# powdr-labs/powdr

Measured on AMD Instinct MI355X. Metric: STARK cells/sec (trace rows x cols) proving guest-keccak [bus interactions (LogUp) inside the proof], higher is better.
Workload: dtype u32 (BabyBear, Montgomery)

## Files before the change

powdr_amd/csrc/babybear.hpp:

```cpp
#pragma once
#if defined(__HIPCC_RTC__)
using __hip_internal::int32_t;
using __hip_internal::int64_t;
using __hip_internal::uint8_t;
using __hip_internal::uint32_t;
using __hip_internal::uint64_t;
#else
#include <stdint.h>
#endif

#if defined(__HIPCC__)
#if !defined(__HIPCC_RTC__)
#include <hip/hip_runtime.h>
#endif
#define PW_HD __host__ __device__ __forceinline__
#else
#define PW_HD inline
#endif

namespace bb {

constexpr uint32_t P = 0x78000001u;
constexpr uint32_t NEG_PINV = 0x77ffffffu;
constexpr uint32_t R_MOD_P = 0x0ffffffeu;
// ... 19 lines not shown
    uint32_t m = (uint32_t)t * NEG_PINV;
    uint64_t u = t + (uint64_t)m * P;
    return (uint32_t)(u >> 32);
}
PW_HD uint32_t add_loose(uint32_t a, uint32_t b) { return reduce_2p(a + b); }
PW_HD uint32_t mul(uint32_t a, uint32_t b) { return monty_reduce((uint64_t)a * b); }
PW_HD uint32_t mul2(uint32_t a, uint32_t b, uint32_t c, uint32_t d) { return monty_reduce((uint64_t)a * b + (uint64_t)c * d); }
PW_HD uint32_t sqr(uint32_t a) { return mul(a, a); }

PW_HD uint32_t to_monty(uint32_t canonical) { return mul(canonical, R2_MOD_P); }
PW_HD uint32_t from_monty(uint32_t x) { return monty_reduce((uint64_t)x); }

PW_HD uint32_t mul_lazy(uint32_t a, uint32_t b) {
    uint64_t t = (uint64_t)a * b;
    uint32_t m = (uint32_t)t * NEG_PINV;
    uint64_t u = t + (uint64_t)m * P;
    return (uint32_t)(u >> 32);
}

PW_HD uint64_t wide_add(uint64_t acc, uint32_t x) {
#if defined(__HIP_DEVICE_COMPILE__)
    uint64_t out;
    asm("v_mad_u64_u32 %0, vcc, %1, 1, %2" : "=v"(out) : "v"(x), "v"(acc) : "vcc");
    return out;
#else
    return acc + x;
#endif
}
PW_HD uint64_t wide_fma(uint64_t acc, uint32_t x, uint32_t k) {
#if defined(__HIP_DEVICE_COMPILE__)
    uint64_t out;
    asm("v_mad_u64_u32 %0, vcc, %1, %2, %3" : "=v"(out) : "v"(x), "n"(k), "v"(acc) : "vcc");
    return out;
#else
    return acc + (uint64_t)x * k;
#endif
}
PW_HD uint64_t wide_fma_uniform(uint64_t c, uint32_t x, uint32_t k) {
#if defined(__HIP_DEVICE_COMPILE__)
    uint64_t out;
    asm("v_mad_u64_u32 %0, vcc, %1, %2, %3" : "=v"(out) : "v"(x), "n"(k), "s"(c) : "vcc");
    return out;
#else
    return c + (uint64_t)x * k;
#endif
}
PW_HD uint64_t wide_mad_uniform(uint64_t acc, uint32_t x, uint32_t u) {
#if defined(__HIP_DEVICE_COMPILE__)
    uint64_t out;
    asm("v_mad_u64_u32 %0, vcc, %1, %2, %3" : "=v"(out) : "v"(x), "s"(u), "v"(acc) : "vcc");
    return out;
#else
    return acc + (uint64_t)x * u;
#endif
}
PW_HD uint64_t wide_mul(uint32_t x, uint32_t k) {
#if defined(__HIP_DEVICE_COMPILE__)
    uint64_t out;
    asm("v_mad_u64_u32 %0, vcc, %1, %2, 0" : "=v"(out) : "v"(x), "n"(k) : "vcc");
    return out;
#else
    return (uint64_t)x * k;
#endif
}
PW_HD uint32_t reduce_wide_loose(uint64_t x) {
    const uint32_t q = (uint32_t)(((x >> 7) & 0xffffffffull) * 273u >> 32);
#if defined(__HIP_DEVICE_COMPILE__) && !defined(PW_NO_REDUCE_MAD)
    uint64_t out;
    asm("v_mad_u64_u32 %0, vcc, %1, %2, %3" : "=v"(out) : "v"(q), "s"(0u - P), "v"(x) : "vcc");
    return (uint32_t)out;
#else
    return (uint32_t)x - q * P;
#endif
}
PW_HD uint32_t reduce_wide(uint64_t x) { return reduce_2p(reduce_wide_loose(x)); }
PW_HD uint32_t reduce_sum(uint64_t x) {
    const uint32_t q = (uint32_t)(x >> 31);
    return reduce_2p((uint32_t)x - q * P);
}

PW_HD int64_t smul(int32_t a, int32_t b) {
#if defined(__HIP_DEVICE_COMPILE__)
    int64_t out;
    asm("v_mad_i64_i32 %0, vcc, %1, %2, 0" : "=v"(out) : "v"(a), "v"(b) : "vcc");
    return out;
#else
    return (int64_t)a * b;
#endif
}
PW_HD int64_t smul_uniform(int32_t a, int32_t u) {
#if defined(__HIP_DEVICE_COMPILE__)
    int64_t out;
    asm("v_mad_i64_i32 %0, vcc, %1, %2, 0" : "=v"(out) : "v"(a), "s"(u) : "vcc");
    return out;
#else
    return (int64_t)a * u;
#endif
}
PW_HD int32_t smont(int64_t t) {
    const int32_t m = (int32_t)((uint32_t)t * NEG_PINV);
#if defined(__HIP_DEVICE_COMPILE__)
    int64_t u;
    asm("v_mad_i64_i32 %0, vcc, %1, %2, %3" : "=v"(u) : "v"(m), "s"((int32_t)P), "v"(t) : "vcc");
    return (int32_t)(u >> 32);
#else
    return (int32_t)((t + (int64_t)m * (int64_t)P) >> 32);
#endif
}
PW_HD int64_t swide_add(int64_t acc, int32_t x) {
#if defined(__HIP_DEVICE_COMPILE__)
    int64_t out;
    asm("v_mad_i64_i32 %0, vcc, %1, 1, %2" : "=v"(out) : "v"(x), "v"(acc) : "vcc");
    return out;
#else
    return acc + x;
#endif
}
PW_HD int64_t swide_fma(int64_t acc, int32_t x, int32_t k) {
#if defined(__HIP_DEVICE_COMPILE__)
    int64_t out;
    asm("v_mad_i64_i32 %0, vcc, %1, %2, %3" : "=v"(out) : "v"(x), "n"(k), "v"(acc) : "vcc");
    return out;
#else
    return acc + (int64_t)x * k;
#endif
}
PW_HD int64_t swide_fma_uniform(int64_t c, int32_t x, int32_t k) {
#if defined(__HIP_DEVICE_COMPILE__)
    int64_t out;
    asm("v_mad_i64_i32 %0, vcc, %1, %2, %3" : "=v"(out) : "v"(x), "n"(k), "s"(c) : "vcc");
    return out;
#else
    return c + (int64_t)x * k;
#endif
}
PW_HD int64_t swide_mad_uniform(int64_t acc, int32_t x, int32_t u) {
#if defined(__HIP_DEVICE_COMPILE__)
    int64_t out;
    asm("v_mad_i64_i32 %0, vcc, %1, %2, %3" : "=v"(out) : "v"(x), "s"(u), "v"(acc) : "vcc");
    return out;
#else
    return acc + (int64_t)x * u;
#endif
}
PW_HD int64_t swide_mul(int32_t x, int32_t k) {
#if defined(__HIP_DEVICE_COMPILE__)
    int64_t out;
    asm("v_mad_i64_i32 %0, vcc, %1, %2, 0" : "=v"(out) : "v"(x), "n"(k) : "vcc");
    return out;
#else
    return (int64_t)x * k;
#endif
}
PW_HD int32_t sreduce_wide_loose(int64_t y) {
    const int32_t a = (int32_t)(y >> 7);
    const int32_t q = (int32_t)(((int64_t)a * 273) >> 32);
#if defined(__HIP_DEVICE_COMPILE__)
    int64_t out;
    asm("v_mad_i64_i32 %0, vcc, %1, %2, %3" : "=v"(out) : "v"(q), "s"(-(int32_t)P), "v"(y) : "vcc");
    return (int32_t)out;
#else
    return (int32_t)((uint32_t)y - (uint32_t)q * P);
#endif
}
PW_HD int32_t centred(uint32_t canonical) { return canonical > P / 2 ? (int32_t)(canonical - P) : (int32_t)canonical; }
PW_HD uint32_t canonical_of(int32_t x) {
    uint32_t u = (uint32_t)x;
    u = umin(u, u + P);
    return umin(u, u - P);
}

constexpr uint32_t TWO_P = 2u * P;
PW_HD uint32_t add_2p(uint32_t a, uint32_t b) {
    const uint32_t s = a + b;
    const uint32_t t = s - TWO_P;
    return s < a ? t : umin(s, t);
}
PW_HD uint32_t sub_2p(uint32_t a, uint32_t b) {
    const uint32_t d = a - b;
    return a < b ? d + TWO_P : d;
}

PW_HD uint32_t double_(uint32_t a) { return add(a, a); }
PW_HD uint32_t halve(uint32_t a) {
    uint32_t t = (a & 1u) ? a + P : a;
    return t >> 1;
}

PW_HD uint32_t pow_u32(uint32_t a, uint32_t e) {
    uint32_t r = R_MOD_P;
    while (e) {
        if (e & 1u) r = mul(r, a);
        a = sqr(a);
        e >>= 1;
    }
    return r;
}

PW_HD uint32_t inv(uint32_t a) {
    uint32_t x2 = sqr(a);
    uint32_t x3 = mul(x2, a);
    uint32_t x6 = sqr(x3);
    uint32_t x7 = mul(x6, a);
    uint32_t o3 = x7;
    uint32_t o6 = o3;
    for (int i = 0; i < 3; ++i) o6 = sqr(o6);
    o6 = mul(o6, o3);
    uint32_t o12 = o6;
    for (int i = 0; i < 6; ++i) o12 = sqr(o12);
    o12 = mul(o12, o6);
    uint32_t o24 = o12;
    for (int i = 0; i < 12; ++i) o24 = sqr(o24);
    o24 = mul(o24, o12);
    uint32_t o27 = o24;
    for (int i = 0; i < 3; ++i) o27 = sqr(o27);
    o27 = mul(o27, o3);
    uint32_t hi = x7;
    for (int i = 0; i < 28; ++i) hi = sqr(hi);
    return mul(hi, o27);
}
PW_HD uint32_t inv_or_zero(uint32_t a) { return a == 0 ? 0u : inv(a); }

}
```

powdr_amd/csrc/ntt.hip:

```cpp
#include "babybear.hpp"
#include "common.hpp"
#include "prover_internal.hpp"

#include <cstdlib>
#include <map>
#include <mutex>
#include <tuple>
#include <type_traits>
#include <vector>

namespace pw {

namespace {

constexpr int kBlock = 256;
__constant__ uint32_t c_roots16[2][8];

__global__ void fill_powers_kernel(uint32_t* out, uint32_t base, uint32_t scale, size_t n) {
    size_t i = (size_t)blockIdx.x * blockDim.x + threadIdx.x;
    if (i < n) out[i] = bb::mul(bb::pow_u32(base, (uint32_t)i), scale);
}
__global__ void bitrev_copy_kernel(const uint32_t* in, uint32_t* out, int n) {
    size_t i = (size_t)blockIdx.x * blockDim.x + threadIdx.x;
    if (i >= ((size_t)1 << n)) return;
// ... 232 lines not shown
                }
            }
        } else {
#pragma unroll
            for (int rho = 0; rho < R; ++rho) tile[p0 + lds_off(rho)] = x[rho];
        }
    }
}

template <bool DIF, int LOGT, int MODE, bool TWT = false>
__global__ __launch_bounds__(kBlock) void ntt_group_kernel(const uint32_t* __restrict__ in, uint32_t* __restrict__ out,
                                                           size_t in_stride, size_t out_stride, GroupParams gp,
                                                           const uint32_t* __restrict__ tw,
                                                           const uint32_t* __restrict__ scale_br) {
    constexpr int EPT = (1 << LOGT) / kBlock;
    __shared__ uint32_t tile[(1 << LOGT) + ((1 << LOGT) >> 5)];
    const int tid = threadIdx.x;
    IndexMap im;
    im.B = gp.B; im.c = gp.c; im.lowbits = gp.lowbits; im.k = gp.k;
    im.cmask = (1u << gp.c) - 1u;
    im.tile0 = (size_t)blockIdx.x << (LOGT - gp.B);
    im.n_tiles = (size_t)gp.n_tiles;
    const uint32_t* src = in + (size_t)blockIdx.y * in_stride;
    uint32_t* dst = out + (size_t)blockIdx.y * out_stride;
    uint32_t tw_base = TWT ? 0u : load_twiddle_base<DIF>(im, gp, 0, 0, tid, tw);
    constexpr bool kStageFold = MODE == 2;
    const bool select = MODE == 2 && gp.n_sel > 0;
    if (kStageFold) {
        if (gp.B == LOGT && gp.c == 0 && gp.lowbits == 0 && gp.fold <= 1) {
            const size_t g0 = (size_t)blockIdx.x << LOGT;
            constexpr int kVec = (1 << LOGT) / (4 * kBlock);
            if (gp.fold == 0) {
                const uint4* pv = reinterpret_cast<const uint4*>(src + g0);
                uint4 d[kVec];
#pragma unroll
                for (int m = 0; m < kVec; ++m) d[m] = pv[(uint32_t)tid + kBlock * m];
                const uint32_t k0 = gp.foldk[0];
#pragma unroll
                for (int m = 0; m < kVec; ++m) {
                    const uint32_t l = 4u * ((uint32_t)tid + kBlock * m);
                    tile[lds_phys(l)] = bb::mul(d[m].x, k0); tile[lds_phys(l + 1)] = bb::mul(d[m].y, k0);
                    tile[lds_phys(l + 2)] = bb::mul(d[m].z, k0); tile[lds_phys(l + 3)] = bb::mul(d[m].w, k0);
                }
            } else {
                const uint4* pv = reinterpret_cast<const uint4*>(src + 2 * g0);
                uint4 d[2 * kVec];
#pragma unroll
                for (int m = 0; m < 2 * kVec; ++m) d[m] = pv[(uint32_t)tid + kBlock * m];
                const uint32_t k0 = gp.foldk[0], k1 = gp.foldk[1];
#pragma unroll
                for (int m = 0; m < 2 * kVec; ++m) {
                    const uint32_t l = 2u * ((uint32_t)tid + kBlock * m);
                    tile[lds_phys(l)] = bb::mul2(d[m].x, k0, d[m].y, k1);
                    tile[lds_phys(l + 1)] = bb::mul2(d[m].z, k0, d[m].w, k1);
                }
            }
        } else {
#pragma unroll 4
            for (uint32_t l = (uint32_t)tid; l < (1u << LOGT); l += kBlock) {
                bool valid;
                const size_t g = im.global(l, valid);
                tile[lds_phys(l)] = valid ? fold_load(src, gp.foldk, g, gp.fold) : 0u;
            }
        }
        __syncthreads();
    }
    for (int r = 0; r < gp.n_rounds; ++r) {
        switch (gp.logr[r]) {
            case 1: run_round<DIF, 1, EPT, MODE, TWT>(tile, im, gp, r, src, dst, tw, scale_br, tid, tw_base, !kStageFold, !select); break;
            case 2: run_round<DIF, 2, EPT, MODE, TWT>(tile, im, gp, r, src, dst, tw, scale_br, tid, tw_base, !kStageFold, !select); break;
            case 3: run_round<DIF, 3, EPT, MODE, TWT>(tile, im, gp, r, src, dst, tw, scale_br, tid, tw_base, !kStageFold, !select); break;
            default: run_round<DIF, 4, EPT, MODE, TWT>(tile, im, gp, r, src, dst, tw, scale_br, tid, tw_base, !kStageFold, !select); break;
        }
        if (r + 1 < gp.n_rounds) __syncthreads();
    }
    if (select) {
        __syncthreads();
        const size_t t = blockIdx.x;
        uint32_t* part = gp.sel_part ? gp.sel_part + ((size_t)blockIdx.y * gp.n_tiles + t) * (size_t)gp.n_sel : nullptr;
        for (int q = tid; q < gp.n_sel; q += kBlock) {
            const uint32_t v = bb::reduce_2p(tile[lds_phys(gp.sel_pos[q])]);
            const uint32_t term = bb::mul(v, gp.sel_xpow[(size_t)q * gp.n_tiles + t]);
            if (part) part[q] = term;
            else atomicAdd(gp.sel_acc + (size_t)blockIdx.y * gp.n_sel + q, (unsigned long long)term);
        }
    }
}

template <bool DIF, int EPT, bool TWT = false>
__device__ __forceinline__ void run_group(uint32_t* tile, const IndexMap& im, const GroupParams& gp, const uint32_t* __restrict__ src,
                                          uint32_t* __restrict__ dst, const uint32_t* __restrict__ tw, int tid, bool io_first, bool io_last) {
    uint32_t tw_base = TWT ? 0u : load_twiddle_base<DIF>(im, gp, 0, 0, tid, tw);
    for (int r = 0; r < gp.n_rounds; ++r) {
        switch (gp.logr[r]) {
            case 1: run_round<DIF, 1, EPT, 0, TWT>(tile, im, gp, r, src, dst, tw, nullptr, tid, tw_base, io_first, io_last); break;
            case 2: run_round<DIF, 2, EPT, 0, TWT>(tile, im, gp, r, src, dst, tw, nullptr, tid, tw_base, io_first, io_last); break;
            case 3: run_round<DIF, 3, EPT, 0, TWT>(tile, im, gp, r, src, dst, tw, nullptr, tid, tw_base, io_first, io_last); break;
            default: run_round<DIF, 4, EPT, 0, TWT>(tile, im, gp, r, src, dst, tw, nullptr, tid, tw_base, io_first, io_last); break;
        }
        if (r + 1 < gp.n_rounds) __syncthreads();
    }
}

__global__ __launch_bounds__(kBlock) void lde_fused_kernel(const uint32_t* __restrict__ in, uint32_t* __restrict__ out, size_t in_stride,
                                                           size_t out_stride, GroupParams ga, GroupParams gd,
                                                           const uint32_t* __restrict__ tw_inv, const uint32_t* __restrict__ tw_fwd,
                                                           const uint32_t* __restrict__ scale_br) {
    constexpr int LOGA = 12, LOGD = 13;
    __shared__ uint32_t tile[(1 << LOGD) + ((1 << LOGD) >> 5)];
    const int tid = threadIdx.x;
    const uint32_t* src = in + (size_t)blockIdx.y * in_stride;
    uint32_t* dst = out + (size_t)blockIdx.y * out_stride;
    IndexMap ia;
    ia.B = ga.B; ia.c = ga.c; ia.lowbits = ga.lowbits; ia.k = ga.k;
    ia.cmask = (1u << ga.c) - 1u;
    ia.tile0 = (size_t)blockIdx.x << (LOGA - ga.B);
    ia.n_tiles = (size_t)ga.n_tiles;
    run_group<true, (1 << LOGA) / kBlock, true>(tile, ia, ga, src, nullptr, tw_inv, tid, true, false);
    __syncthreads();
    uint32_t v[(1 << LOGA) / kBlock];
#pragma unroll
    for (int m = 0; m < (1 << LOGA) / kBlock; ++m) {
        const uint32_t l = (uint32_t)tid + 256u * m;
        bool valid;
        const size_t q = ia.global(l, valid);
        const uint32_t sc = valid ? scale_br[q] : 0u;
        v[m] = bb::mul(tile[lds_phys(l)], sc);
    }
    __syncthreads();
#pragma unroll
    for (int m = 0; m < (1 << LOGA) / kBlock; ++m) {
        const uint32_t l = (uint32_t)tid + 256u * m;
        tile[lds_phys(2 * l)] = v[m];
        tile[lds_phys(2 * l + 1)] = v[m];
    }
    __syncthreads();
    IndexMap id;
    id.B = gd.B; id.c = gd.c; id.lowbits = gd.lowbits; id.k = gd.k;
    id.cmask = (1u << gd.c) - 1u;
    id.tile0 = (size_t)blockIdx.x << (LOGD - gd.B);
    id.n_tiles = (size_t)gd.n_tiles;
    run_group<false, (1 << LOGD) / kBlock, true>(tile, id, gd, nullptr, dst, tw_fwd, tid, false, true);
}

constexpr uint32_t kF12A0 = 0, kF12A1 = 15u * 256u, kF12A2 = kF12A1 + 15u * 16u;
constexpr uint32_t kF12D0 = 4096, kF12D1 = kF12D0 + 15u * 2u, kF12D2 = kF12D1 + 15u * 32u;
constexpr uint32_t kF12Words = kF12D2 + 15u * 512u;

template <int RB>
__device__ constexpr uint32_t f12_off(int rho) {
    return ((uint32_t)rho << RB) + (RB >= 5 ? ((uint32_t)rho << (RB >= 5 ? RB - 5 : 0)) : ((uint32_t)rho >> (RB >= 5 ? 0 : 5 - RB)));
}

template <bool CANON>
__global__ __launch_bounds__(kBlock) void lde_fused12_kernel(const uint32_t* __restrict__ in, uint32_t* __restrict__ out, size_t in_stride,
                                                             size_t out_stride, const uint32_t* __restrict__ tw, uint32_t hinv) {
    __shared__ uint32_t tile[(1 << 13) + ((1 << 13) >> 5)];
    const uint32_t tid = threadIdx.x;
    const uint32_t* src = in + (size_t)blockIdx.y * in_stride + ((size_t)blockIdx.x << 12);
    uint32_t* dst = out + (size_t)blockIdx.y * out_stride + ((size_t)blockIdx.x << 13);
    uint32_t x[16], tt[16], tn[16];
#pragma unroll
    for (int rho = 0; rho < 16; ++rho) x[rho] = src[tid + 256u * rho];
#pragma unroll
    for (int j = 0; j < 15; ++j) tt[j] = tw[kF12A0 + 256u * j + tid];
#pragma unroll
    for (int j = 0; j < 15; ++j) tn[j] = tw[kF12A1 + 16u * j + (tid & 15u)];
    slot_butterflies<true, 4, true>(x, 0u, tt);
    {
        const uint32_t p0 = lds_phys(tid);
#pragma unroll
        for (int rho = 0; rho < 16; ++rho) tile[p0 + f12_off<8>(rho)] = x[rho];
    }
    __syncthreads();
    {
        const uint32_t k = ((tid >> 5) & 1u) | (((tid >> 4) & 1u) << 1) | ((tid >> 6) << 2);
        const uint32_t p0 = lds_phys((k << 8) | (tid & 15u));
#pragma unroll
        for (int rho = 0; rho < 16; ++rho) x[rho] = tile[p0 + f12_off<4>(rho)];
        slot_butterflies<true, 4, true>(x, 0u, tn);
#pragma unroll
        for (int rho = 0; rho < 16; ++rho) tile[p0 + f12_off<4>(rho)] = x[rho];
    }
    __syncthreads();
    {
        const uint32_t p0 = lds_phys(tid << 4);
#pragma unroll
        for (int rho = 0; rho < 16; ++rho) x[rho] = tile[p0 + (uint32_t)rho];
#pragma unroll
        for (int j = 0; j < 15; ++j) tn[j] = tw[kF12D1 + 32u * j + (tid & 31u)];
#pragma unroll
        for (int j = 0; j < 15; ++j) tt[j] = tw[kF12A2 + j];
        slot_butterflies<true, 4, true>(x, 0u, tt);
#pragma unroll
        for (int rho = 0; rho < 16; ++rho) x[rho] = bb::mul(x[rho], hinv);
    }
    __syncthreads();
    {
        const uint32_t p0 = lds_phys(tid << 5);
#pragma unroll
        for (int b = 0; b < 2; ++b) {
            uint32_t y[16];
#pragma unroll
            for (int rho = 0; rho < 16; ++rho) y[rho] = x[rho];
#pragma unroll
            for (int j = 0; j < 15; ++j) tt[j] = tw[kF12D0 + 2u * j + b];
            slot_butterflies<false, 4, true>(y, 0u, tt);
#pragma unroll
            for (int rho = 0; rho < 16; ++rho) tile[p0 + 2u * rho + b] = y[rho];
        }
    }
    __syncthreads();
    uint32_t tf[2][16];
#pragma unroll
    for (int m = 0; m < 2; ++m) {
#pragma unroll
        for (int j = 0; j < 15; ++j) tf[m][j] = tw[kF12D2 + 512u * j + tid + 256u * m];
    }
#pragma unroll
    for (int m = 0; m < 2; ++m) {
        const uint32_t sigma = tid + 256u * m;
        const uint32_t p0 = lds_phys(((sigma >> 5) << 9) | (sigma & 31u));
#pragma unroll
        for (int rho = 0; rho < 16; ++rho) x[rho] = tile[p0 + f12_off<5>(rho)];
        slot_butterflies<false, 4, true>(x, 0u, tn);
#pragma unroll
        for (int rho = 0; rho < 16; ++rho) tile[p0 + f12_off<5>(rho)] = x[rho];
    }
    __syncthreads();
#pragma unroll
    for (int m = 0; m < 2; ++m) {
        const uint32_t sigma = tid + 256u * m;
        const uint32_t p0 = lds_phys(sigma);
#pragma unroll
        for (int rho = 0; rho < 16; ++rho) x[rho] = tile[p0 + f12_off<9>(rho)];
        slot_butterflies<false, 4, true>(x, 0u, tf[m]);
#pragma unroll
        for (int rho = 0; rho < 16; ++rho) dst[sigma + 512u * rho] = CANON ? bb::reduce_2p(x[rho]) : x[rho];
    }
}

template <int RB>
__device__ __forceinline__ constexpr uint32_t strided8_words(int lb, int m, int rho) {
    return RB == 9 ? (((uint32_t)(8 * m) << lb) + ((uint32_t)rho << (lb + 4))) : (((uint32_t)m << (lb + 7)) + ((uint32_t)rho << lb));
}
typedef __attribute__((address_space(1))) const char* GlobalBytesIn;
typedef __attribute__((address_space(1))) char* GlobalBytesOut;
__device__ __forceinline__ uint32_t ld_off4(const uint32_t* base, uint32_t off4) {
    GlobalBytesIn b = (GlobalBytesIn)base;
    asm("" : "+s"(b));
    return *(__attribute__((address_space(1))) const uint32_t*)(b + off4);
}
__device__ __forceinline__ void st_off4(uint32_t* base, uint32_t off4, uint32_t v) {
    GlobalBytesOut b = (GlobalBytesOut)base;
    asm("" : "+s"(b));
    *(__attribute__((address_space(1))) uint32_t*)(b + off4) = v;
}

template <bool DIF, int K>
__global__ __launch_bounds__(kBlock) void ntt_strided_kernel(const uint32_t* in, uint32_t* out, size_t in_stride, size_t out_stride,
                                                             const uint32_t* __restrict__ tw, uint32_t cst_lo, uint32_t cst_hi) {
    static_assert(K == 8, "the 2^20-row geometry; other heights take ntt_group_kernel");
    constexpr int LB = DIF ? 12 : 13;
    constexpr int RB0 = DIF ? 9 : 5, RB1 = DIF ? 5 : 9;
    __shared__ uint32_t tile[(1 << 13) + ((1 << 13) >> 5)];
    const uint32_t tid = threadIdx.x, row = tid >> 5, col = tid & 31u;
    const size_t t0 = (size_t)blockIdx.x << 5;
    const uint32_t* src = in + (size_t)blockIdx.y * in_stride + t0;
    uint32_t* dst = out + (size_t)blockIdx.y * out_stride + t0;
    const uint32_t off_hi = 4u * ((row << LB) | col), off_lo = 4u * ((row << (LB + 4)) | col);
    const uint32_t off0 = RB0 == 9 ? off_hi : off_lo, off1 = RB1 == 9 ? off_hi : off_lo;
    uint32_t x[2][16];
#pragma unroll
    for (int m = 0; m < 2; ++m) {
#pragma unroll
        for (int rho = 0; rho < 16; ++rho) x[m][rho] = ld_off4(src + strided8_words<RB0>(LB, m, rho), off0);
    }
    uint32_t b_hi[2], b_lo;
#pragma unroll
    for (int m = 0; m < 2; ++m) b_hi[m] = ld_off4(tw + t0 + ((uint32_t)(8 * m) << LB), off_hi);
    b_lo = ld_off4(tw + (t0 << 4), col << 6);
    if (!DIF) {
        b_lo = bb::mul(b_lo, cst_lo);
#pragma unroll
        for (int m = 0; m < 2; ++m) b_hi[m] = bb::mul(b_hi[m], cst_hi);
    }
    const uint32_t p_hi = lds_phys(tid), p_lo = (row << 9) + (row << 4) + col;
    const uint32_t p0 = RB0 == 9 ? p_hi : p_lo, p1 = RB1 == 9 ? p_hi : p_lo;
    constexpr uint32_t kSlot0 = RB0 == 9 ? 264u : 4224u, kSlot1 = RB1 == 9 ? 264u : 4224u;
#pragma unroll
    for (int m = 0; m < 2; ++m) {
        slot_butterflies<DIF, 4>(x[m], RB0 == 9 ? b_hi[m] : b_lo);
#pragma unroll
        for (int rho = 0; rho < 16; ++rho) tile[p0 + kSlot0 * m + f12_off<RB0>(rho)] = x[m][rho];
    }
    __syncthreads();
#pragma unroll
    for (int m = 0; m < 2; ++m) {
        uint32_t y[16];
#pragma unroll
        for (int rho = 0; rho < 16; ++rho) y[rho] = tile[p1 + kSlot1 * m + f12_off<RB1>(rho)];
        slot_butterflies<DIF, 4>(y, RB1 == 9 ? b_hi[m] : b_lo);
#pragma unroll
        for (int rho = 0; rho < 16; ++rho) st_off4(dst + strided8_words<RB1>(LB, m, rho), off1, DIF ? y[rho] : bb::reduce_2p(y[rho]));
    }
}

struct Tables {
    uint32_t* tw_fwd = nullptr;
    uint32_t* tw_inv = nullptr;
    uint32_t* shift = nullptr;
    uint32_t* shift_br = nullptr;
};
std::mutex g_mu;
std::map<std::pair<int, int>, Tables> g_tables;
uint64_t g_roots_uploaded = 0;

int upload_roots() {
    int device = 0;
    PW_HIP_TRY(hipGetDevice(&device));
    if (device < 64 && (g_roots_uploaded >> device) & 1) return 0;
    uint32_t h[2][8];
    const uint32_t w16 = field::root_of_unity(4), w16i = bb::inv(w16);
    uint32_t a = bb::R_MOD_P, b = bb::R_MOD_P;
    for (int r = 0; r < 8; ++r) { h[0][r] = a; h[1][r] = b; a = bb::mul(a, w16); b = bb::mul(b, w16i); }
    PW_HIP_TRY(hipMemcpyToSymbol(HIP_SYMBOL(c_roots16), h, sizeof h));
    if (device < 64) g_roots_uploaded |= 1ull << device;
    return 0;
}

const Tables* tables(int n) {
    std::lock_guard<std::mutex> lk(g_mu);
    if (upload_roots()) return nullptr;
    int device = 0;
    if (hipGetDevice(&device) != hipSuccess) return nullptr;
    const std::pair<int, int> key{device, n};
    auto it = g_tables.find(key);
    if (it != g_tables.end()) return &it->second;
    Tables t;
    size_t half = n ? (size_t)1 << (n - 1) : 1, full = (size_t)1 << n;
    if (hipMalloc(&t.tw_fwd, half * 4) != hipSuccess) return nullptr;
    if (hipMalloc(&t.tw_inv, half * 4) != hipSuccess) return nullptr;
    if (hipMalloc(&t.shift, full * 4) != hipSuccess) return nullptr;
    if (hipMalloc(&t.shift_br, full * 4) != hipSuccess) return nullptr;
    uint32_t w = field::root_of_unity(n);
    uint32_t one = bb::R_MOD_P;
    hipLaunchKernelGGL(fill_powers_kernel, dim3(div_up(half, 256)), dim3(256), 0, stream(), t.tw_fwd, w, one, half);
    hipLaunchKernelGGL(fill_powers_kernel, dim3(div_up(half, 256)), dim3(256), 0, stream(), t.tw_inv, bb::inv(w), one, half);
    uint32_t ninv = bb::inv(bb::to_monty((uint32_t)(((uint64_t)1 << n) % bb::P)));
    hipLaunchKernelGGL(fill_powers_kernel, dim3(div_up(full, 256)), dim3(256), 0, stream(), t.shift,
                       bb::to_monty(field::kCosetShift), ninv, full);
    hipLaunchKernelGGL(bitrev_copy_kernel, dim3(div_up(full, 256)), dim3(256), 0, stream(), t.shift, t.shift_br, n);
    if (hipStreamSynchronize(stream()) != hipSuccess) return nullptr;
    return &g_tables.emplace(key, t).first->second;
}

GroupParams make_group(bool dif, int n, int s, int k, int c) {
    GroupParams g{};
    g.n = n; g.s0 = s; g.k = k; g.c = c; g.lowbits = dif ? n - s - k : s; g.B = k + c;
    g.n_tiles = 1ull << (n - g.B);
    int nr = (k + 3) / 4;
    g.n_rounds = nr;
    int widths[4];
    for (int r = 0; r < nr; ++r) widths[r] = k / nr + (r < k % nr ? 1 : 0);
    if (dif) {
        int top = c + k;
        for (int r = 0; r < nr; ++r) { top -= widths[r]; g.rb[r] = top; g.logr[r] = widths[r]; }
    } else {
        int bot = c;
        for (int r = 0; r < nr; ++r) { g.rb[r] = bot; g.logr[r] = widths[r]; bot += widths[r]; }
    }
    return g;
}

std::vector<GroupParams> plan_groups(bool dif, int n, int first, int& logt_out, int end = -1, bool balance = false) {
    std::vector<GroupParams> out;
    int kStridedC = (n - (dif ? 0 : 1)) >= 18 ? 5 : 4;
    if (const char* e = getenv("POWDR_NTT_C")) { int v = atoi(e); if (v >= 0 && v <= 6) kStridedC = v; }
    if (end < 0) end = n;
    const int total = end - first;
    int logt = 12;
    int n_groups = 0;
    {
        auto passes = [&](int lt) {
            int s = first, p = 0;
            while (s < end) {
                int rem = end - s, k = rem < lt ? rem : lt;
                for (; k >= 1; --k) { int lb = dif ? n - s - k : s; int c = lb < kStridedC ? lb : kStridedC; if (k + c <= lt) break; }
                s += k; ++p;
            }
            return p;
// ... 76 lines not shown
    const unsigned j = (i - a.off[r]) >> a.rb[r];
    const int q = 31 - __clz((int)(j + 1));
    out[i] = bb::mul(tab[i], a.cq[r][q]);
}

struct CosetSpec {
    int fold_log;
    uint32_t foldk[16];
    uint32_t C[32];
    uint32_t* d_scratch;
    int n_sel = 0;
    const uint32_t* sel_pos = nullptr;
    const uint32_t* sel_xpow = nullptr;
    unsigned long long* sel_acc = nullptr;
    uint32_t* sel_part = nullptr;
};

template <class Launch>
void for_column_chunks(uint32_t cols, Launch&& launch) {
    for (uint32_t c0 = 0; c0 < cols; c0 += 65535u) launch(c0, cols - c0 < 65535u ? cols - c0 : 65535u);
}

template <bool DIF>
void launch_group_kernel(int logt, int mode, dim3 grid, const uint32_t* src, uint32_t* dst, size_t src_stride, size_t dst_stride,
                         const GroupParams& g, const uint32_t* table, const uint32_t* tw, const uint32_t* scale_br) {
    auto launch = [&](auto lt, auto md) {
        constexpr int LT = decltype(lt)::value, MD = decltype(md)::value;
        if (table) hipLaunchKernelGGL((ntt_group_kernel<DIF, LT, MD, true>), grid, dim3(kBlock), 0, stream(), src, dst, src_stride, dst_stride, g, table, scale_br);
        else hipLaunchKernelGGL((ntt_group_kernel<DIF, LT, MD, false>), grid, dim3(kBlock), 0, stream(), src, dst, src_stride, dst_stride, g, tw, scale_br);
    };
    auto with_mode = [&](auto lt) {
        if constexpr (!DIF) {
            if (mode == 2) return launch(lt, std::integral_constant<int, 2>{});
            if (mode == 1) return launch(lt, std::integral_constant<int, 1>{});
        }
        launch(lt, std::integral_constant<int, 0>{});
    };
    if (logt == 13) with_mode(std::integral_constant<int, 13>{});
    else with_mode(std::integral_constant<int, 12>{});
}

template <bool DIF>
bool strided8_geometry(const GroupParams& g, int logt) {
    return logt == 13 && g.n == (DIF ? 20 : 21) && g.s0 == (DIF ? 0 : 13) && g.k == 8 && g.c == 5 && g.lowbits == (DIF ? 12 : 13) && g.B == 13 &&
           g.n_tiles == (DIF ? 128ull : 256ull) && g.n_rounds == 2 && g.logr[0] == 4 && g.logr[1] == 4 && g.rb[0] == (DIF ? 9 : 5) &&
           g.rb[1] == (DIF ? 5 : 9) && (DIF || g.canonical_out) && !g.fold && !g.n_sel;
}

template <bool DIF>
void launch_groups(std::vector<GroupParams>& groups, int logt, int mode, const uint32_t* in, uint32_t* out, size_t in_stride, size_t out_stride,
                   uint32_t cols, const uint32_t* tw, const uint32_t* expand_scale_br, const char* name, const CosetSpec* cs = nullptr,
                   const uint32_t* coset_pw = nullptr, bool fused_schedule = false) {
    const uint32_t* src = in;
    size_t src_stride = in_stride;
    for (auto& g : groups) {
        const unsigned wgs = (unsigned)div_up((size_t)g.n_tiles, (size_t)1 << (logt - g.B));
        const GroupTwiddles* gt = group_twiddles(g, DIF);
        if (gt) for (int r = 0; r < 4; ++r) g.twt_off[r] = gt->off[r];
        const uint32_t* table = gt ? gt->d : nullptr;
        if (coset_pw) {
            g.coset = 1;
            for (int r = 0; r < g.n_rounds; ++r) g.cst[r] = coset_pw[g.n - 1 - (g.s0 + g.rb[r] + g.logr[r] - 1 - g.c)];
        }
        if (cs) {
            g.coset = 1;
            g.fold = mode == 2 ? cs->fold_log : 0;
            for (int k = 0; k < 16; ++k) g.foldk[k] = cs->foldk[k];
            if (mode == 2 && cs->n_sel > 0) { g.n_sel = cs->n_sel; g.sel_pos = cs->sel_pos; g.sel_xpow = cs->sel_xpow; g.sel_acc = cs->sel_acc; g.sel_part = cs->sel_part; }
            for (int r = 0; r < g.n_rounds; ++r) g.cst[r] = cs->C[g.s0 + g.rb[r] + g.logr[r] - 1 - g.c];
            if (gt) {
                CosetTableArgs a{};
                a.n_rounds = g.n_rounds;
                for (int r = 0; r < g.n_rounds; ++r) {
                    a.off[r] = gt->off[r]; a.rb[r] = g.rb[r]; a.logr[r] = g.logr[r];
                    for (int q = 0; q < g.logr[r]; ++q) a.cq[r][q] = cs->C[g.s0 + g.rb[r] - g.c + q];
                }
                const int lr = g.n_rounds - 1;
                a.total = gt->off[lr] + (((1u << g.logr[lr]) - 1u) << g.rb[lr]);
                hipLaunchKernelGGL(coset_table_kernel, dim3(div_up(a.total, 256)), dim3(256), 0, stream(), gt->d, cs->d_scratch, a);
                table = cs->d_scratch;
            }
        }
        if (fused_schedule && mode == 0 && !table && !cs && strided8_geometry<DIF>(g, logt)) {
            const uint32_t one = bb::R_MOD_P;
            const uint32_t cst_lo = g.coset ? g.cst[DIF ? 1 : 0] : one, cst_hi = g.coset ? g.cst[DIF ? 0 : 1] : one;
            for_column_chunks(cols, [&](uint32_t c0, uint32_t cc) {
                ScopedKernelTimer t(name);
                call_stats()[kStatNttStridedFixedLaunches] += 1;
                hipLaunchKernelGGL((ntt_strided_kernel<DIF, 8>), dim3((unsigned)g.n_tiles, cc), dim3(kBlock), 0, stream(), src + (size_t)c0 * src_stride,
                                   out + (size_t)c0 * out_stride, src_stride, out_stride, tw, cst_lo, cst_hi);
            });
            src = out;
            src_stride = out_stride;
            continue;
        }
        for_column_chunks(cols, [&](uint32_t c0, uint32_t cc) {
            ScopedKernelTimer t(mode == 2 ? "ntt_subcoset_first_group_kernel" : name);
            launch_group_kernel<DIF>(logt, mode, dim3(wgs, cc), src + (size_t)c0 * src_stride, out + (size_t)c0 * out_stride, src_stride, out_stride,
                                     g, table, tw, expand_scale_br);
        });
        src = out;
        src_stride = out_stride;
        mode = 0;
        expand_scale_br = nullptr;
    }
}

template <bool DIF>
void run_groups(const uint32_t* in, uint32_t* out, size_t in_stride, size_t out_stride, uint32_t cols, int n,
                int first_stage, const uint32_t* tw, const uint32_t* expand_scale_br, const char* name, const CosetSpec* cs = nullptr,
                int max_groups = -1, int* stages_done = nullptr) {
    int logt = 12;
    auto groups = plan_groups(DIF, n, first_stage, logt);
    if (max_groups >= 0 && (size_t)max_groups < groups.size()) groups.resize((size_t)max_groups);
    if (stages_done) { *stages_done = first_stage; for (auto& g : groups) *stages_done += g.k; }
    const bool complete = !stages_done || *stages_done == n;
    if (!groups.empty() && complete) groups.back().canonical_out = 1;
    launch_groups<DIF>(groups, logt, cs ? 2 : expand_scale_br != nullptr ? 1 : 0, in, out, in_stride, out_stride, cols, tw, expand_scale_br, name, cs);
    if (groups.empty() && in != out) {
        for (uint32_t c = 0; c < cols; ++c)
            (void)hipMemcpyAsync(out + (size_t)c * out_stride, in + (size_t)c * in_stride, (size_t)4 << n,
                                 hipMemcpyDeviceToDevice, stream());
    }
}

__global__ void expand_small_kernel(const uint32_t* in, uint32_t* out, size_t in_stride, size_t out_stride, size_t h,
                                    const uint32_t* scale_br) {
    size_t q = (size_t)blockIdx.x * blockDim.x + threadIdx.x;
    if (q >= h) return;
    uint32_t v = bb::mul(in[(size_t)blockIdx.y * in_stride + q], scale_br[q]);
    out[(size_t)blockIdx.y * out_stride + 2 * q] = v;
    out[(size_t)blockIdx.y * out_stride + 2 * q + 1] = v;
}

struct FusedTwiddles {
    uint32_t* d = nullptr;
    unsigned dif_off[4] = {0, 0, 0, 0}, dit_off[4] = {0, 0, 0, 0};
    size_t dit_base = 0;
};
std::map<std::pair<int, int>, FusedTwiddles> g_fused_tw;

const FusedTwiddles* fused_twiddles(int ka, const GroupParams& ga, const GroupParams& gd) {
    return cached_table(g_fused_tw, ka, [&](std::vector<uint32_t>& h, FusedTwiddles& ft) {
        append_group_table(h, ga, true, ft.dif_off, 0);
        ft.dit_base = h.size();
        append_group_table(h, gd, false, ft.dit_off, ft.dit_base);
        return true;
    });
}

struct Fused12Twiddles { uint32_t* d = nullptr; };
std::map<std::pair<int, int>, Fused12Twiddles> g_fused12_tw;

const uint32_t* fused12_twiddles(int n, const GroupParams& ga, const GroupParams& gd, const uint32_t* pw) {
    const Fused12Twiddles* ft = cached_table(g_fused12_tw, n, [&](std::vector<uint32_t>& h, Fused12Twiddles&) {
        unsigned dif_off[4] = {0, 0, 0, 0}, dit_off[4] = {0, 0, 0, 0};
        append_group_table(h, ga, true, dif_off, 0);
        if (h.size() > kF12D0) return false;
        h.resize(kF12D0, 0u);
        append_group_table(h, gd, false, dit_off, kF12D0);
        if (dif_off[0] != kF12A0 || dif_off[1] != kF12A1 || dif_off[2] != kF12A2 || dit_off[0] != 0 || kF12D0 + dit_off[1] != kF12D1 ||
            kF12D0 + dit_off[2] != kF12D2 || h.size() != kF12Words)
            return false;
        for (int r = 0; r < gd.n_rounds; ++r) {
            const size_t G = (size_t)1 << gd.rb[r];
            uint32_t* tab = h.data() + kF12D0 + dit_off[r];
            for (int q = 0; q < gd.logr[r]; ++q) {
                const uint32_t cq = pw[n - (gd.s0 + gd.rb[r] - gd.c + q)];
                for (size_t i = (((size_t)1 << q) - 1) * G; i < (((size_t)2 << q) - 1) * G; ++i) tab[i] = bb::mul(tab[i], cq);
            }
        }
        return true;
    });
    return ft ? ft->d : nullptr;
}

}

int lde_fused(const uint32_t* in, uint32_t* tmp, uint32_t* out, size_t in_stride, size_t tmp_stride, size_t out_stride, uint32_t cols, int n) {
    if (n == 0) {
        int rc = intt_dif(in, tmp, in_stride, tmp_stride, cols, n);
        return rc ? rc : coset_lde_from_coeffs(tmp, out, tmp_stride, out_stride, cols, n);
    }
    const Tables* tn = tables(n);
    const Tables* t1 = tables(n + 1);
    if (!tn || !t1) return (int)hipErrorOutOfMemory;
    const int ka = n < 12 ? n : 12;
    const char* force_generic = getenv("POWDR_LDE_FUSED_GENERIC");
    const bool spec12 = ka == 12 && !(force_generic && atoi(force_generic) != 0);
    const char* strided_generic = getenv("POWDR_NTT_STRIDED_GENERIC");
    const bool strided_fixed = !(strided_generic && atoi(strided_generic) != 0);
    const uint32_t hinv = bb::inv(bb::to_monty((uint32_t)(((uint64_t)1 << n) % bb::P)));
    const uint32_t* src = in;
    size_t src_stride = in_stride;
    if (n > ka) {
        int logt = 12;
        auto groups = plan_groups(true, n, 0, logt, n - ka, true);
        launch_groups<true>(groups, logt, 0, in, tmp, in_stride, tmp_stride, cols, tn->tw_inv, nullptr, "ntt_group_kernel<dif>", nullptr, nullptr,
                            strided_fixed);
        src = tmp;
        src_stride = tmp_stride;
    }
    GroupParams ga = make_group(true, n, n - ka, ka, 0);
    GroupParams gd = make_group(false, n + 1, 1, ka, 1);
    gd.canonical_out = ka == n ? 1 : 0;
    uint32_t coset_pw[33];
    if (spec12) {
        coset_pw[0] = bb::to_monty(field::kCosetShift);
        for (int e = 1; e <= n; ++e) coset_pw[e] = bb::sqr(coset_pw[e - 1]);
        const uint32_t* tw12 = fused12_twiddles(n, ga, gd, coset_pw);
        if (!tw12) return (int)hipErrorOutOfMemory;
        const unsigned wgs = 1u << (n - 12);
        for_column_chunks(cols, [&](uint32_t c0, uint32_t cc) {
            ScopedKernelTimer t("lde_fused_kernel");
            const uint32_t* s_ = src + (size_t)c0 * src_stride;
            uint32_t* d_ = out + (size_t)c0 * out_stride;
            if (n == 12) hipLaunchKernelGGL(lde_fused12_kernel<true>, dim3(wgs, cc), dim3(kBlock), 0, stream(), s_, d_, src_stride, out_stride, tw12, hinv);
            else hipLaunchKernelGGL(lde_fused12_kernel<false>, dim3(wgs, cc), dim3(kBlock), 0, stream(), s_, d_, src_stride, out_stride, tw12, hinv);
        });
    } else {
        const FusedTwiddles* ft = fused_twiddles(ka, ga, gd);
        if (!ft) return (int)hipErrorOutOfMemory;
        for (int r = 0; r < 4; ++r) { ga.twt_off[r] = ft->dif_off[r]; gd.twt_off[r] = ft->dit_off[r]; }
        const unsigned wgs = (unsigned)div_up((size_t)ga.n_tiles, (size_t)1 << (12 - ka));
        for_column_chunks(cols, [&](uint32_t c0, uint32_t cc) {
            ScopedKernelTimer t("lde_fused_kernel");
            hipLaunchKernelGGL(lde_fused_kernel, dim3(wgs, cc), dim3(kBlock), 0, stream(), src + (size_t)c0 * src_stride,
                               out + (size_t)c0 * out_stride, src_stride, out_stride, ga, gd, ft->d, ft->d + ft->dit_base, tn->shift_br);
        });
    }
    if (n > ka) {
        int logt = 12;
        auto groups = plan_groups(false, n + 1, ka + 1, logt, n + 1, true);
        if (!groups.empty()) groups.back().canonical_out = 1;
        launch_groups<false>(groups, logt, 0, out, out, out_stride, out_stride, cols, t1->tw_fwd, nullptr, "ntt_group_kernel<dit>", nullptr,
                             spec12 ? coset_pw : nullptr, strided_fixed);
    }
    return (int)hipGetLastError();
}

int intt_dif(const uint32_t* in, uint32_t* out, size_t in_stride, size_t out_stride, uint32_t cols, int n) {
    const Tables* t = tables(n);
    if (!t) return (int)hipErrorOutOfMemory;
    run_groups<true>(in, out, in_stride, out_stride, cols, n, 0, t->tw_inv, nullptr, "ntt_group_kernel<dif>");
    return (int)hipGetLastError();
}

int coset_lde_from_coeffs(const uint32_t* coeffs, uint32_t* out, size_t in_stride, size_t out_stride, uint32_t cols, int n) {
    const Tables* tn = tables(n);
    const Tables* t1 = tables(n + 1);
    if (!tn || !t1) return (int)hipErrorOutOfMemory;
    if (n == 0) {
        ScopedKernelTimer t("expand_small_kernel");
        hipLaunchKernelGGL(expand_small_kernel, dim3(1, cols), dim3(64), 0, stream(), coeffs, out, in_stride, out_stride,
                           (size_t)1, tn->shift_br);
        return (int)hipGetLastError();
    }
    run_groups<false>(coeffs, out, in_stride, out_stride, cols, n + 1, 1, t1->tw_fwd, tn->shift_br, "ntt_group_kernel<dit>");
    return (int)hipGetLastError();
}

namespace {
bool subcoset_spec(int n, int b, uint32_t r, uint32_t* d_scratch, CosetSpec& cs) {
    const int nm = n + 1 - b;
    if (b < 1 || b > 5 || nm < 1 || (r >> b)) return false;
    cs = CosetSpec{};
    cs.fold_log = b - 1;
    cs.d_scratch = d_scratch;
    uint32_t pw[32];
    pw[0] = bb::mul(bb::to_monty(field::kCosetShift), bb::pow_u32(field::root_of_unity(n + 1), r));
    for (int e = 1; e <= nm; ++e) pw[e] = bb::sqr(pw[e - 1]);
    for (int s = 0; s < nm; ++s) cs.C[s] = pw[nm - 1 - s];
    const uint32_t hinv = bb::inv(bb::to_monty((uint32_t)(((uint64_t)1 << n) % bb::P)));
    const int f = b - 1;
    for (uint32_t tp = 0; tp < (1u << f); ++tp) {
        const uint32_t t = f ? (__builtin_bitreverse32(tp) >> (32 - f)) : 0u;
        cs.foldk[tp] = bb::mul(bb::pow_u32(pw[nm], t), hinv);
    }
    return true;
}

__global__ __launch_bounds__(256) void subcoset_rows_kernel(const uint32_t* __restrict__ part, size_t stride, uint32_t cols, int k1, int k2, uint32_t c0,
                                                            uint32_t wm, const uint32_t* __restrict__ idx, const uint32_t* __restrict__ slot,
                                                            uint32_t* __restrict__ out) {
    const uint32_t c = blockIdx.x * 256u + threadIdx.x;
    if (c >= cols) return;
    const uint32_t i = idx[blockIdx.y];
    const uint32_t x = bb::mul(c0, bb::pow_u32(wm, i));
    const uint32_t* col = part + (size_t)c * stride + (i & ((1u << k1) - 1u));
    uint32_t acc = 0u, xp = bb::R_MOD_P;
    for (uint32_t u = 0; u < (1u << k2); ++u) {
        const uint32_t t = k2 ? (__brev(u) >> (32 - k2)) : 0u;
        acc = bb::add(acc, bb::mul(bb::reduce_2p(col[(size_t)t << k1]), xp));
        xp = bb::mul(xp, x);
    }
    out[(size_t)(slot ? slot[blockIdx.y] : blockIdx.y) * cols + c] = acc;
}
__global__ __launch_bounds__(256) void select_xpow_kernel(const uint32_t* __restrict__ idx, uint32_t n_idx, int k2, uint32_t c0, uint32_t wm,
                                                         uint32_t* __restrict__ xpow, uint32_t* __restrict__ pos, uint32_t pos_mask) {
    const size_t gid = (size_t)blockIdx.x * 256 + threadIdx.x;
    const size_t n_tiles = (size_t)1 << k2;
    if (gid >= (size_t)n_idx * n_tiles) return;
    const uint32_t q = (uint32_t)(gid >> k2), t = (uint32_t)(gid & (n_tiles - 1));
    const uint32_t i = idx[q];
    const uint32_t x = bb::mul(c0, bb::pow_u32(wm, i));
    const uint32_t u = k2 ? (__brev(t) >> (32 - k2)) : 0u;
    xpow[gid] = bb::pow_u32(x, u);
    if (t == 0) pos[q] = i & pos_mask;
}

__global__ __launch_bounds__(256) void select_finish_kernel(const unsigned long long* __restrict__ acc, uint32_t n, uint32_t cols,
                                                           const uint32_t* __restrict__ slot, uint32_t* __restrict__ out) {
    const uint32_t c = blockIdx.x * 256u + threadIdx.x;
    if (c >= cols) return;
    const uint32_t q = blockIdx.y;
    out[(size_t)(slot ? slot[q] : q) * cols + c] = (uint32_t)(acc[(size_t)c * n + q] % bb::P);
}
__global__ __launch_bounds__(128) void select_reduce_kernel(const uint32_t* __restrict__ part, uint32_t n, uint32_t cols, size_t n_tiles,
                                                           const uint32_t* __restrict__ slot, uint32_t* __restrict__ out) {
    const uint32_t q = blockIdx.x * 128u + threadIdx.x, c = blockIdx.y;
    if (q >= n) return;
    const uint32_t* col = part + (size_t)c * n_tiles * n + q;
    unsigned long long acc = 0;
#pragma unroll 8
    for (size_t t = 0; t < n_tiles; ++t) acc += col[t * n];
    out[(size_t)(slot ? slot[q] : q) * cols + c] = (uint32_t)(acc % bb::P);
}
}

int subcoset_query_rows(const uint32_t* coeffs, size_t in_stride, uint32_t cols, int n, int b, uint32_t r, const uint32_t* d_local_idx,
                        uint32_t n_idx, const uint32_t* d_slot, uint32_t* rows_out, uint32_t* d_work, size_t work_words) {
    const int nm = n + 1 - b;
    if (!n_idx || !cols) return 0;
    if (cols > 65535u) return 1;
    const int sel_mode = getenv("POWDR_QUERY_SELECT") ? atoi(getenv("POWDR_QUERY_SELECT")) : 1;
    if (sel_mode == 0) return 1;
    CosetSpec cs;
    if (!subcoset_spec(n, b, r, d_work, cs)) return (int)hipErrorInvalidValue;
    int logt = 12;
    auto groups = plan_groups(false, nm, 0, logt);
    if (groups.size() < 2 || logt != 12 || groups[0].B != 12 || groups[0].c != 0 || groups[0].lowbits != 0 || cs.fold_log > 1) return 1;
    const int k1 = groups[0].k, k2 = nm - k1;
    const size_t n_tiles = (size_t)1 << k2;
    uint32_t* d_pos = d_work + (1u << 13);
    uint32_t* d_xpow = d_pos + ((n_idx + 1u) & ~1u);
    unsigned long long* d_acc = reinterpret_cast<unsigned long long*>(d_xpow + (((size_t)n_idx * n_tiles + 1) & ~(size_t)1));
    uint32_t* d_part = reinterpret_cast<uint32_t*>(d_acc + (size_t)cols * n_idx);
    bool partial = sel_mode != 2;
    size_t need = (size_t)(d_part - d_work) + (partial ? (size_t)cols * n_tiles * n_idx : 0);
    if (partial && need > work_words) { partial = false; need = (size_t)(d_part - d_work); }
    if (need > work_words || ((uintptr_t)d_work & 7)) return 1;
    const Tables* tm = tables(nm);
    if (!tm) return (int)hipErrorOutOfMemory;
    const uint32_t c0 = bb::mul(bb::to_monty(field::kCosetShift), bb::pow_u32(field::root_of_unity(n + 1), r));
    {
        ScopedKernelTimer t("subcoset_rows_kernel");
        hipLaunchKernelGGL(select_xpow_kernel, dim3((unsigned)div_up((size_t)n_idx * n_tiles, 256)), dim3(256), 0, stream(), d_local_idx, n_idx, k2, c0,
                           field::root_of_unity(nm), d_xpow, d_pos, (1u << k1) - 1u);
    }
    if (!partial) PW_HIP_TRY(hipMemsetAsync(d_acc, 0, (size_t)cols * n_idx * sizeof(unsigned long long), stream()));
    cs.n_sel = (int)n_idx; cs.sel_pos = d_pos; cs.sel_xpow = d_xpow; cs.sel_acc = d_acc; cs.sel_part = partial ? d_part : nullptr;
    int done = 0;
    run_groups<false>(coeffs, const_cast<uint32_t*>(coeffs), in_stride, in_stride, cols, nm, 0, tm->tw_fwd, nullptr, "ntt_group_kernel<dit>", &cs, 1, &done);
    {
        ScopedKernelTimer t("subcoset_rows_kernel");
        if (partial) hipLaunchKernelGGL(select_reduce_kernel, dim3(div_up(n_idx, 128), cols), dim3(128), 0, stream(), d_part, n_idx, cols, n_tiles, d_slot, rows_out);
        else hipLaunchKernelGGL(select_finish_kernel, dim3(div_up(cols, 256), n_idx), dim3(256), 0, stream(), d_acc, n_idx, cols, d_slot, rows_out);
    }
    return (int)hipGetLastError();
}

// ... 49 lines not shown
```

Baseline: 7.179 billion.

## Use signed Montgomery DIT butterflies and fold hinv into twiddles in fused12 LDE

The forward (DIT) stages of the 12-bit fused LDE kernel now use signed Montgomery butterflies on centred twiddles. Each butterfly computes a*kappa + b*w and a*kappa - b*w and reduces both with smont. The separate per-element multiply by the inverse size (hinv) is removed: it is folded into the first-stage kappa and into the precomputed first-layer twiddles on the host. Outputs are turned back to canonical form with a cheap single conditional add, and static asserts check that the value range closes across stages. The aim is fewer modular multiplies and reductions per element. The risks are a subtle correctness dependency on those range bounds and a behaviour change: outputs are now always canonical, including for n > 12.

```diff
diff --git a/powdr_amd/csrc/babybear.hpp b/powdr_amd/csrc/babybear.hpp
--- a/powdr_amd/csrc/babybear.hpp
+++ b/powdr_amd/csrc/babybear.hpp
@@ -195,6 +195,13 @@
     return (int64_t)x * k;
 #endif
 }
+PW_HD void dit_signed(int32_t& a, int32_t& b, int32_t w, int32_t nw, int32_t kappa = (int32_t)R_MOD_P) {
+    const int64_t ak = smul_uniform(a, kappa);
+    const int64_t tx = ak + (int64_t)b * w, ty = ak + (int64_t)b * nw;
+    a = smont(tx);
+    b = smont(ty);
+}
+PW_HD uint32_t canonical_of_centred(int32_t x) { return umin((uint32_t)x, (uint32_t)x + P); }
 PW_HD int32_t sreduce_wide_loose(int64_t y) {
     const int32_t a = (int32_t)(y >> 7);
     const int32_t q = (int32_t)(((int64_t)a * 273) >> 32);
diff --git a/powdr_amd/csrc/ntt.hip b/powdr_amd/csrc/ntt.hip
--- a/powdr_amd/csrc/ntt.hip
+++ b/powdr_amd/csrc/ntt.hip
@@ -408,14 +408,45 @@
     return ((uint32_t)rho << RB) + (RB >= 5 ? ((uint32_t)rho << (RB >= 5 ? RB - 5 : 0)) : ((uint32_t)rho >> (RB >= 5 ? 0 : 5 - RB)));
 }
 
-template <bool CANON>
+namespace ntt {
+namespace bounds {
+constexpr int64_t kSmontDomain = 4899916392431616000ll;
+constexpr int64_t kInTop = 2013265921ll;
+constexpr int64_t kTwiddleTop = 1006632960ll;
+constexpr int64_t kWideTop = 4053239664633446400ll;
+constexpr int64_t kOutTop = 1950351361ll;
+static_assert(kSmontDomain == (int64_t)((1ull << 63) - ((uint64_t)bb::P << 31)), "smont's domain");
+static_assert(kInTop == (int64_t)bb::P && kTwiddleTop == (int64_t)(bb::P - 1) / 2, "B = 1, centred twiddles");
+static_assert(kWideTop == 2 * (kInTop - 1) * kTwiddleTop && kWideTop < kSmontDomain, "a kappa + b w stays inside smont's domain");
+static_assert(kOutTop == (int64_t)(((uint64_t)kWideTop + ((uint64_t)bb::P << 31)) >> 32) + 1, "the reduction adds at most 2^31 p");
+static_assert(kOutTop <= kInTop, "the range closes: outputs are inputs of the next stage");
+static_assert(kOutTop + (int64_t)bb::P <= (1ll << 32), "canonical_of_centred: x + p does not wrap for x >= 0");
+static_assert((int64_t)bb::R_MOD_P <= kTwiddleTop, "kappa = R mod p is centred as it stands");
+}
+}
+
+__device__ __forceinline__ void slot_dit_signed(int32_t* v, const int32_t* tt, int32_t kappa0) {
+#pragma unroll
+    for (int q = 0; q < 4; ++q) {
+#pragma unroll
+        for (int u = 0; u < 8; ++u) {
+            const int lowp = u & ((1 << q) - 1);
+            const int i0 = ((u >> q) << (q + 1)) | lowp;
+            const int i1 = i0 | (1 << q);
+            const int32_t w = tt[(1 << q) - 1 + lowp];
+            bb::dit_signed(v[i0], v[i1], w, -w, q == 0 ? kappa0 : (int32_t)bb::R_MOD_P);
+        }
+    }
+}
+
 __global__ __launch_bounds__(kBlock) void lde_fused12_kernel(const uint32_t* __restrict__ in, uint32_t* __restrict__ out, size_t in_stride,
-                                                             size_t out_stride, const uint32_t* __restrict__ tw, uint32_t hinv) {
+                                                             size_t out_stride, const uint32_t* __restrict__ tw, int32_t hinv_c) {
     __shared__ uint32_t tile[(1 << 13) + ((1 << 13) >> 5)];
     const uint32_t tid = threadIdx.x;
     const uint32_t* src = in + (size_t)blockIdx.y * in_stride + ((size_t)blockIdx.x << 12);
     uint32_t* dst = out + (size_t)blockIdx.y * out_stride + ((size_t)blockIdx.x << 13);
     uint32_t x[16], tt[16], tn[16];
+    int32_t te[16];
 #pragma unroll
     for (int rho = 0; rho < 16; ++rho) x[rho] = src[tid + 256u * rho];
 #pragma unroll
@@ -444,44 +475,42 @@
 #pragma unroll
         for (int rho = 0; rho < 16; ++rho) x[rho] = tile[p0 + (uint32_t)rho];
 #pragma unroll
-        for (int j = 0; j < 15; ++j) tn[j] = tw[kF12D1 + 32u * j + (tid & 31u)];
+        for (int j = 0; j < 15; ++j) te[j] = (int32_t)tw[kF12D1 + 32u * j + (tid & 31u)];
 #pragma unroll
         for (int j = 0; j < 15; ++j) tt[j] = tw[kF12A2 + j];
         slot_butterflies<true, 4, true>(x, 0u, tt);
-#pragma unroll
-        for (int rho = 0; rho < 16; ++rho) x[rho] = bb::mul(x[rho], hinv);
     }
     __syncthreads();
     {
         const uint32_t p0 = lds_phys(tid << 5);
 #pragma unroll
         for (int b = 0; b < 2; ++b) {
-            uint32_t y[16];
-#pragma unroll
-            for (int rho = 0; rho < 16; ++rho) y[rho] = x[rho];
-#pragma unroll
-            for (int j = 0; j < 15; ++j) tt[j] = tw[kF12D0 + 2u * j + b];
-            slot_butterflies<false, 4, true>(y, 0u, tt);
-#pragma unroll
-            for (int rho = 0; rho < 16; ++rho) tile[p0 + 2u * rho + b] = y[rho];
+            int32_t y[16], ts[16];
+#pragma unroll
+            for (int rho = 0; rho < 16; ++rho) y[rho] = (int32_t)x[rho];
+#pragma unroll
+            for (int j = 0; j < 15; ++j) ts[j] = (int32_t)tw[kF12D0 + 2u * j + b];
+            slot_dit_signed(y, ts, hinv_c);
+#pragma unroll
+            for (int rho = 0; rho < 16; ++rho) tile[p0 + 2u * rho + b] = (uint32_t)y[rho];
         }
     }
     __syncthreads();
-    uint32_t tf[2][16];
+    int32_t tf[2][16], sx[16];
 #pragma unroll
     for (int m = 0; m < 2; ++m) {
 #pragma unroll
-        for (int j = 0; j < 15; ++j) tf[m][j] = tw[kF12D2 + 512u * j + tid + 256u * m];
+        for (int j = 0; j < 15; ++j) tf[m][j] = (int32_t)tw[kF12D2 + 512u * j + tid + 256u * m];
     }
 #pragma unroll
     for (int m = 0; m < 2; ++m) {
         const uint32_t sigma = tid + 256u * m;
         const uint32_t p0 = lds_phys(((sigma >> 5) << 9) | (sigma & 31u));
 #pragma unroll
-        for (int rho = 0; rho < 16; ++rho) x[rho] = tile[p0 + f12_off<5>(rho)];
-        slot_butterflies<false, 4, true>(x, 0u, tn);
-#pragma unroll
-        for (int rho = 0; rho < 16; ++rho) tile[p0 + f12_off<5>(rho)] = x[rho];
+        for (int rho = 0; rho < 16; ++rho) sx[rho] = (int32_t)tile[p0 + f12_off<5>(rho)];
+        slot_dit_signed(sx, te, (int32_t)bb::R_MOD_P);
+#pragma unroll
+        for (int rho = 0; rho < 16; ++rho) tile[p0 + f12_off<5>(rho)] = (uint32_t)sx[rho];
     }
     __syncthreads();
 #pragma unroll
@@ -489,10 +518,10 @@
         const uint32_t sigma = tid + 256u * m;
         const uint32_t p0 = lds_phys(sigma);
 #pragma unroll
-        for (int rho = 0; rho < 16; ++rho) x[rho] = tile[p0 + f12_off<9>(rho)];
-        slot_butterflies<false, 4, true>(x, 0u, tf[m]);
-#pragma unroll
-        for (int rho = 0; rho < 16; ++rho) dst[sigma + 512u * rho] = CANON ? bb::reduce_2p(x[rho]) : x[rho];
+        for (int rho = 0; rho < 16; ++rho) sx[rho] = (int32_t)tile[p0 + f12_off<9>(rho)];
+        slot_dit_signed(sx, tf[m], (int32_t)bb::R_MOD_P);
+#pragma unroll
+        for (int rho = 0; rho < 16; ++rho) dst[sigma + 512u * rho] = bb::canonical_of_centred(sx[rho]);
     }
 }
 
@@ -875,7 +904,7 @@
 struct Fused12Twiddles { uint32_t* d = nullptr; };
 std::map<std::pair<int, int>, Fused12Twiddles> g_fused12_tw;
 
-const uint32_t* fused12_twiddles(int n, const GroupParams& ga, const GroupParams& gd, const uint32_t* pw) {
+const uint32_t* fused12_twiddles(int n, const GroupParams& ga, const GroupParams& gd, const uint32_t* pw, uint32_t hinv) {
     const Fused12Twiddles* ft = cached_table(g_fused12_tw, n, [&](std::vector<uint32_t>& h, Fused12Twiddles&) {
         unsigned dif_off[4] = {0, 0, 0, 0}, dit_off[4] = {0, 0, 0, 0};
         append_group_table(h, ga, true, dif_off, 0);
@@ -889,8 +918,9 @@
             const size_t G = (size_t)1 << gd.rb[r];
             uint32_t* tab = h.data() + kF12D0 + dit_off[r];
             for (int q = 0; q < gd.logr[r]; ++q) {
-                const uint32_t cq = pw[n - (gd.s0 + gd.rb[r] - gd.c + q)];
-                for (size_t i = (((size_t)1 << q) - 1) * G; i < (((size_t)2 << q) - 1) * G; ++i) tab[i] = bb::mul(tab[i], cq);
+                uint32_t cq = pw[n - (gd.s0 + gd.rb[r] - gd.c + q)];
+                if (r == 0 && q == 0) cq = bb::mul(cq, hinv);
+                for (size_t i = (((size_t)1 << q) - 1) * G; i < (((size_t)2 << q) - 1) * G; ++i) tab[i] = (uint32_t)bb::centred(bb::mul(tab[i], cq));
             }
         }
         return true;
@@ -931,15 +961,14 @@
     if (spec12) {
         coset_pw[0] = bb::to_monty(field::kCosetShift);
         for (int e = 1; e <= n; ++e) coset_pw[e] = bb::sqr(coset_pw[e - 1]);
-        const uint32_t* tw12 = fused12_twiddles(n, ga, gd, coset_pw);
+        const uint32_t* tw12 = fused12_twiddles(n, ga, gd, coset_pw, hinv);
         if (!tw12) return (int)hipErrorOutOfMemory;
         const unsigned wgs = 1u << (n - 12);
         for_column_chunks(cols, [&](uint32_t c0, uint32_t cc) {
             ScopedKernelTimer t("lde_fused_kernel");
             const uint32_t* s_ = src + (size_t)c0 * src_stride;
             uint32_t* d_ = out + (size_t)c0 * out_stride;
-            if (n == 12) hipLaunchKernelGGL(lde_fused12_kernel<true>, dim3(wgs, cc), dim3(kBlock), 0, stream(), s_, d_, src_stride, out_stride, tw12, hinv);
-            else hipLaunchKernelGGL(lde_fused12_kernel<false>, dim3(wgs, cc), dim3(kBlock), 0, stream(), s_, d_, src_stride, out_stride, tw12, hinv);
+            hipLaunchKernelGGL(lde_fused12_kernel, dim3(wgs, cc), dim3(kBlock), 0, stream(), s_, d_, src_stride, out_stride, tw12, bb::centred(hinv));
         });
     } else {
         const FusedTwiddles* ft = fused_twiddles(ka, ga, gd);
```

Result: faster. 7.264 billion, median of 6 (+1.2%).
